# zhengchen1999/DOVE

Measured on AMD Instinct MI355X. Metric: SR frames/s (33x720x1280 4x one-step, whole job), higher is better.
Workload: dtype bf16; 1 GPU; synthetic 33x720x1280 HR clip (LR 180x320, 4x), one-step t=399, CogVideoX1.5-5B VAE + 42-layer DiT random-init, 1 clip per GPU (BASELINE configs[1]); weight_sums=True, vae_streams=2, variant=headline (bf16)

## Files before the change

### dove_amd/csrc/graph.hip

```cpp
#include <dlfcn.h>
#include <math.h>
#include <stdio.h>
#include <stdlib.h>
#include <string.h>

#include <algorithm>
#include <map>
#include <string>
#include <unordered_map>
#include <vector>

#include "common.h"
#include "../../include/dove_hip.h"
#include "ctx_access.h"

namespace {

#define CHK(expr)            \
  do {                       \
    const int rc__ = (expr); \
    if (rc__ != 0) return rc__; \
  } while (0)
#define HIPCHK(expr)                                                              \
  do {                                                                            \
// ... 689 lines not shown
      if (k) ++active;
    }
    return active;
  }
  int r = 0;
  for (int i = 0; i < nb; ++i) {
    const int s = fb[i].first, e = fb[i].second, n = e - s;
    const int spare = (world - r) - (nb - i);
    int head; bool can;
    if (enc) { head = (n % 2) + 4 * ((n - n % 2) / 8); can = n - (n % 2) >= 8 && (n - n % 2) % 8 == 0; }
    else { head = n - 1; can = n >= 2; }
    if (spare >= 1 && can) {
      const bool odd = n % 2 == 1;
      (*out)[r].push_back({s, s + head, odd ? 1 : 2, r + 1, true});
      (*out)[r + 1].push_back({s + head, e, 2, r, false});
      r += 2;
    } else {
      (*out)[r].push_back({s, e, 0, -1, false});
      r += 1;
    }
  }
  return r;
}
int piece_out_frames(const dove_ctx* c, bool enc, int t, int role) {
  if (role == 0) return enc ? enc_batch_frames(c, t) : dec_batch_frames(c, t);
  for (int i = 0; i < n_temporal_stages(c); ++i) {
    if (enc) t = t > 1 ? (t % 2 ? 1 + (t - 1) / 2 : t / 2) : 1;
    else t = role == 1 ? 2 * t - 1 : 2 * t;
  }
  return t;
}
struct RankPlan { std::vector<Piece> mine; std::vector<int> out_first; int active = 1; int total_out = 0; std::vector<int> rank_first, rank_count; };
void rank_plan(const dove_ctx* c, bool enc, int n, RankPlan* rp) {
  std::vector<std::pair<int, int>> fb;
  frame_batches(n, enc ? c->cfg.vae_enc_batch : c->cfg.vae_dec_batch, &fb);
  std::vector<std::vector<Piece>> plan;
  rp->active = plan_pieces(fb, c->nranks, enc, &plan);
  rp->rank_first.assign(c->nranks, 0); rp->rank_count.assign(c->nranks, 0);
  int f = 0;
  for (int r = 0; r < c->nranks; ++r) {
    rp->rank_first[r] = f;
    for (auto& pc : plan[r]) {
      const int k = piece_out_frames(c, enc, pc.e - pc.s, pc.role);
      if (r == c->rank) { rp->mine.push_back(pc); rp->out_first.push_back(f); }
      rp->rank_count[r] += k;
      f += k;
    }
  }
  rp->total_out = f;
}
void set_piece(dove_ctx* c, const Piece* pc) {
  c->piece_role = pc ? pc->role : 0; c->piece_partner = pc ? pc->partner : -1; c->piece_lower = pc ? pc->lower : false;
}
int norm_silu(dove_ctx* c, const Tensor& x, float* fused_stats, const std::string& name, const Tensor* zq, Tensor* out, void* stream) {
  const float eps = c->cfg.vae_norm_eps;
  float* stats = fused_stats;
  const int nb = c->nb, Ti = x.T / nb;
  if (c->piece_partner >= 0) {
    hipStream_t s = (hipStream_t)stream;
    double* sums = (double*)fused_stats;
    if (!sums) {
      sums = (double*)c->arena.alloc(64 * sizeof(double));
      DOVE_CHECK_ARG(sums, "workspace exhausted (GroupNorm sums)");
      CHK(dove_groupnorm_sums_bf16(x.p, x.elems() / x.C, (long long)x.H * x.W, x.C, gn_scratch(c), c->gn_ws_rows, sums, stream));
    }
    double* msg = (double*)c->arena.alloc(3 * 72 * sizeof(double));
    DOVE_CHECK_ARG(msg, "workspace exhausted (GroupNorm pair message)");
    double *mine = msg, *theirs = msg + 72, *tot = msg + 144;
    hipLaunchKernelGGL(gn_msg_kernel, dim3(1), dim3(128), 0, s, sums, (double)(x.elems() / 32), mine);
    CHK(pair_exchange(c, c->piece_partner, c->piece_lower, mine, theirs, 65 * sizeof(double), stream));
    hipLaunchKernelGGL(gn_add_kernel, dim3(1), dim3(128), 0, s, c->piece_lower ? mine : theirs, c->piece_lower ? theirs : mine, tot);
    c->arena.release(sums);
    stats = (float*)c->arena.alloc(64 * 4);
    CHK(dove_groupnorm_finalize_sums(tot, 0.0, eps, stats, stream));
    c->arena.release(msg);
  } else if (!stats) {
    stats = (float*)c->arena.alloc((size_t)nb * 64 * 4);
    CHK(dove_groupnorm_stats_nb_bf16(x.p, nb, x.elems() / x.C / nb, (long long)x.H * x.W, x.C, eps, gn_scratch(c), c->gn_ws_rows, stats, stream));
  }
  const auto& gb = c->aff.at(name);
  CHK(alloc_t(c, x.T, x.H, x.W, x.C, out));
  if (!zq) {
    CHK(dove_groupnorm_apply_nb_bf16(x.p, out->p, nb, Ti, x.H, x.W, x.C, stats, gb.first, gb.second, 1, nullptr, 0, 0, 0, 0, nullptr, stream));
  } else {
    Tensor yb;
    CHK(conv(c, *zq, c->pc.at(name + ".yb"), ConvOpt(), &yb, stream));
    const int ratio = x.H / zq->H;
    int sshift = 0;
    while ((1 << sshift) < ratio) ++sshift;
    std::vector<int> tmap;
    spatial_norm_tmap(Ti, zq->T / nb, &tmap);
    CHK(dove_groupnorm_apply_nb_bf16(x.p, out->p, nb, Ti, x.H, x.W, x.C, stats, gb.first, gb.second, 1, yb.p, zq->T / nb, yb.H, yb.W, sshift,
                                     tmap.data(), stream));
    free_t(c, yb);
  }
  c->arena.release(stats);
  return 0;
}
int resnet(dove_ctx* c, Tensor* x, float** xstats, const std::string& name, const Tensor* zq, void* stream, int tdup = 0) {
  const float eps = c->cfg.vae_norm_eps;
  Tensor h1, h, h2, y;
  CHK(norm_silu(c, *x, *xstats, name + ".norm1", zq, &h1, stream));
  float* hs = nullptr;
  ConvOpt o1; o1.gn_eps = eps; o1.gn_stats = &hs; o1.tdup = tdup;
  CHK(cconv(c, h1, true, name + ".conv1", o1, &h, stream));
  CHK(norm_silu(c, h, hs, name + ".norm2", zq, &h2, stream));
  free_t(c, h);
  Tensor sc = *x;
  bool own_sc = false;
  auto it = c->pc.find(name + ".conv_shortcut");
  if (it != c->pc.end()) { CHK(conv(c, *x, it->second, ConvOpt(), &sc, stream)); own_sc = true; }
  float* ys = nullptr;
  ConvOpt o2; o2.resid = sc.p; o2.ldr = sc.C; o2.gn_eps = eps; o2.gn_stats = &ys;
  CHK(cconv(c, h2, true, name + ".conv2", o2, &y, stream));
  if (own_sc) free_t(c, sc);
  free_t(c, *x);
  *x = y; *xstats = ys;
  return 0;
}
void clear_caches(dove_ctx* c);
struct StageGuard {
  dove_ctx* c;
  explicit StageGuard(dove_ctx* ctx) : c(ctx) {
    if (c && c->depth++ == 0) {
      clear_caches(c); c->arena.reset(); c->halo_recv = c->halo_send = false; c->nb = 1; set_piece(c, nullptr);
      c->ev_next = 0; c->halo_posted.clear(); c->halo_record.clear(); c->halo_sent = false;
      c->vae_multi = false;
    }
  }
  ~StageGuard() { if (c) --c->depth; }
};

int encoder(dove_ctx* c, const Tensor& x, Tensor* out, void* stream) {
  const auto& cf = c->cfg;
  Tensor h; float* hs = nullptr;
  Tensor xin = x;
  CHK(cconv(c, xin, false, c->pc.count("encoder.conv_in.taps") ? "encoder.conv_in.taps" : "encoder.conv_in", ConvOpt(), &h, stream));
  char nm[128];
  const int n_tdown = n_temporal_stages(c);
  for (int i = 0; i < cf.vae_num_blocks; ++i) {
    for (int j = 0; j < cf.vae_layers_per_block; ++j) { snprintf(nm, sizeof nm, "encoder.down_blocks.%d.resnets.%d", i, j); CHK(resnet(c, &h, &hs, nm, nullptr, stream)); }
    if (i < cf.vae_num_blocks - 1) {
      snprintf(nm, sizeof nm, "encoder.down_blocks.%d.downsamplers.0", i);
      if (hs) { c->arena.release(hs); hs = nullptr; }
      Tensor p = h;
      const int Ti = h.T / c->nb;
      if (i < n_tdown && Ti > 1) {
        const int To = Ti % 2 ? 1 + (Ti - 1) / 2 : Ti / 2;
        CHK(alloc_t(c, c->nb * To, h.H, h.W, h.C, &p));
        CHK(dove_avgpool_time_nb_bf16(h.p, c->nb, Ti, (long long)h.H * h.W * h.C, p.p, stream));
        free_t(c, h);
      }
      ConvOpt od; od.stride = 2; od.pad_h = 0; od.pad_w = 0; od.nb = c->nb;
      Tensor d;
      CHK(conv(c, p, c->pc.at(nm), od, &d, stream));
      free_t(c, p);
      h = d;
    }
  }
  for (int j = 0; j < 2; ++j) { snprintf(nm, sizeof nm, "encoder.mid_block.resnets.%d", j); CHK(resnet(c, &h, &hs, nm, nullptr, stream)); }
  Tensor n;
  CHK(norm_silu(c, h, hs, "encoder.norm_out", nullptr, &n, stream));
  free_t(c, h);
  CHK(cconv(c, n, true, "encoder.conv_out", ConvOpt(), out, stream));
  return 0;
}
int decoder(dove_ctx* c, const Tensor& z, Tensor* out, void* stream) {
  const auto& cf = c->cfg;
  Tensor h; float* hs = nullptr;
// ... 1065 lines not shown
```

### dove_amd/lib.py

```python
from __future__ import annotations

import ctypes as C
import os

import torch

_HERE = os.path.dirname(os.path.abspath(__file__))
LIB_PATH = os.path.join(_HERE, "libdove_hip.so")
_lib = None

F32, BF16, U8 = 0, 1, 2
METRIC_PSNR, METRIC_SSIM, METRIC_RGB_TO_Y = 1, 2, 4
COLORFIX_WAVELET, COLORFIX_ADAIN, COLORFIX_CLAMP = 1, 2, 1
YUV_444, YUV_422, YUV_420, YUV_MONO = 0, 1, 2, 3
YUV_SITING_LEFT, YUV_SITING_CENTRE = 0, 1
VIDEO_RGB_U8, VIDEO_YUV = 0, 1
RESIZE_BILINEAR, RESIZE_BICUBIC, RESIZE_AREA = 0, 1, 2
ACT_NONE, ACT_RELU, ACT_SIGMOID, ACT_TANH = 0, 1, 2, 3


class ConvDesc(C.Structure):
    _fields_ = [
        ("struct_size", C.c_uint), ("reserved", C.c_uint),
        ("x", C.c_void_p), ("cache", C.c_void_p), ("w", C.c_void_p), ("bias", C.c_void_p),
# ... 65 lines not shown
                ("x", C.c_void_p), ("w", C.c_void_p), ("bias", C.c_void_p), ("scale", C.c_void_p), ("shift", C.c_void_p), ("out", C.c_void_p),
                ("n", C.c_int), ("h", C.c_int), ("w_in", C.c_int), ("cin", C.c_int), ("cout", C.c_int), ("kh", C.c_int), ("kw", C.c_int),
                ("stride", C.c_int), ("act", C.c_int), ("out_mul", C.c_float), ("ldx", C.c_longlong), ("ldo", C.c_longlong)]

    def __init__(self, *a, **k):
        super().__init__(*a, **k)
        self.struct_size = C.sizeof(Conv2dF32Args)


class ConvnetConvF32Args(C.Structure):
    _fields_ = [("struct_size", C.c_uint), ("reserved", C.c_uint),
                ("x", C.c_void_p), ("w", C.c_void_p), ("bias", C.c_void_p), ("out", C.c_void_p),
                ("n", C.c_int), ("h", C.c_int), ("w_in", C.c_int), ("cin", C.c_int), ("cout", C.c_int), ("kh", C.c_int), ("kw", C.c_int),
                ("stride", C.c_int), ("pad_h", C.c_int), ("pad_w", C.c_int), ("relu", C.c_int), ("reserved2", C.c_int),
                ("ldx", C.c_longlong), ("ldo", C.c_longlong)]

    def __init__(self, *a, **k):
        super().__init__(*a, **k)
        self.struct_size = C.sizeof(ConvnetConvF32Args)


class ResnetConvF32Args(C.Structure):
    _fields_ = [("struct_size", C.c_uint), ("reserved", C.c_uint),
                ("x", C.c_void_p), ("w", C.c_void_p), ("bias", C.c_void_p), ("residual", C.c_void_p), ("out", C.c_void_p),
                ("n", C.c_int), ("h", C.c_int), ("w_in", C.c_int), ("cin", C.c_int), ("cout", C.c_int), ("k", C.c_int),
                ("stride", C.c_int), ("pool", C.c_int), ("relu", C.c_int), ("reserved2", C.c_int),
                ("ldx", C.c_longlong), ("ldr", C.c_longlong), ("ldo", C.c_longlong)]

    def __init__(self, *a, **k):
        super().__init__(*a, **k)
        self.struct_size = C.sizeof(ResnetConvF32Args)


class PreNoise(C.Structure):
    _fields_ = [("eps", C.c_void_p), ("eps_dtype", C.c_int), ("sqrt_alpha", C.c_float), ("sqrt_one_minus_alpha", C.c_float)]


OPT_VAE_TILING, OPT_VAE_SAMPLE_HEIGHT, OPT_VAE_SAMPLE_WIDTH, OPT_DIT_LINEAR_MXFP8, OPT_DIT_ATTN_MXFP8, OPT_WEIGHT_SUMS, OPT_VAE_STREAMS = 1, 2, 3, 4, 5, 6, 7
STAT_HALO_PREPOSTED, STAT_HALO_BLOCKING, STAT_HALO_SENT, STAT_HALO_COMMUNICATORS = 100, 101, 102, 103


_VP, _I, _LL, _F = C.c_void_p, C.c_int, C.c_longlong, C.c_float
_ULL, _PI, _PLL = C.c_ulonglong, C.POINTER(C.c_int), C.POINTER(C.c_longlong)
XFER_FN = C.CFUNCTYPE(C.c_int, C.c_void_p, C.c_int, C.c_void_p, C.c_size_t, C.c_void_p)
GROUP_FN = C.CFUNCTYPE(C.c_int, C.c_void_p, C.c_void_p)

SIGNATURES = {
    "dove_conv_igemm_bf16": [C.POINTER(ConvDesc), _VP],
    "dove_groupnorm_stats_bf16": [_VP, _LL, _LL, _I, _F, _VP, _I, _VP, _VP],
    "dove_groupnorm_finalize_partials": [_VP, _LL, C.c_double, _F, _VP, _VP, _VP],
    "dove_groupnorm_stats_nb_bf16": [_VP, _I, _LL, _LL, _I, _F, _VP, _I, _VP, _VP],
    "dove_groupnorm_finalize_partials_nb": [_VP, _LL, _I, C.c_double, _F, _VP, C.c_size_t, _VP, _VP],
    "dove_groupnorm_apply_nb_bf16": [_VP, _VP, _I, _I, _I, _I, _I, _VP, _VP, _VP, _I, _VP, _I, _I, _I, _I, C.POINTER(C.c_int), _VP],
    "dove_avgpool_time_nb_bf16": [_VP, _I, _I, _LL, _VP, _VP],
    "dove_groupnorm_sums_bf16": [_VP, _LL, _LL, _I, _VP, _I, _VP, _VP],
    "dove_groupnorm_finalize_sums": [_VP, C.c_double, _F, _VP, _VP],
    "dove_groupnorm_sums_from_partials": [_VP, _LL, _VP, _VP, _VP],
    "dove_groupnorm_apply_bf16": [_VP, _VP, _I, _I, _I, _I, _VP, _VP, _VP, _I, _VP, _I, _I, _I, C.POINTER(C.c_int), _VP],
    "dove_layernorm_modulate_bf16": [_VP, _VP, _LL, _I, _F, _VP, _VP, _VP, _LL, _VP],
    "dove_qkv_post_bf16": [_VP, _LL, _LL, _I, _I, _I, _VP, _VP, _VP, _VP, _VP, _VP, _F, _F, _VP, _VP, _VP, _I, _VP, _VP],
    "dove_vt_quad_swap_bf16": [_VP, _LL, _LL, _VP],
    "dove_ulysses_place_bf16": [_VP, _VP, _VP, C.POINTER(C.c_longlong), _I, _I, _LL, _LL, _VP, _VP, _VP, _VP, _VP],
    "dove_cl_im2col3x3_from_ncthw": [_VP, _I, _I, _I, _I, _I, _I, _F, _F, _VP, _VP],
    "dove_conv_out_gather": [_VP, _LL, _I, _I, _I, _I, _VP, _F, _F, _F, _F, _VP, _I, _VP],
    "dove_attention_fwd_bf16": [_VP, _VP, _VP, _VP, _LL, _LL, _I, _I, _LL, _VP, _VP],
    "dove_qkv_post_mxfp8": [_VP, _LL, _LL, _I, _I, _I, _VP, _VP, _VP, _VP, _VP, _VP, _F, _F, _VP, _VP, _VP, _VP, _VP],
    "dove_attention_fwd_mxfp8": [_VP, _VP, _VP, _VP, _VP, _LL, _LL, _I, _I, _LL, _VP],
    "dove_cl_from_ncthw": [_VP, _I, _I, _LL, _I, _F, _F, _VP, _VP],
    "dove_ncthw_from_cl": [_VP, _LL, _I, _LL, _F, _F, _F, _F, _VP, _I, _VP],
    "dove_avgpool_time_bf16": [_VP, _I, _LL, _VP, _VP],
    "dove_posterior_sample": [_VP, _LL, _I, _LL, _VP, _I, _VP, _I, _VP],
    "dove_axpby": [_VP, _VP, _VP, _I, _LL, _F, _F, _VP],
    "dove_patchify": [_VP, _I, _I, _I, _I, _I, _I, _I, _VP, _LL, _VP],
    "dove_unpatchify": [_VP, _LL, _I, _I, _I, _I, _I, _I, _VP, _I, _VP],
    "dove_gemv_bf16": [_VP, _VP, _VP, _I, _I, _I, _VP, _VP],
    "dove_blend_edge_bf16": [_VP, _VP, _I, _I, _I, _I, _I, _I, _I, _I, _VP],
    "dove_preprocess_u8": [_VP, _I, _I, _I, _I, _I, _I, _I, _VP, _I, _VP],
    "dove_postprocess_u8": [_VP, _I, _I, _I, _I, _I, _I, _I, _VP, _VP],
    "dove_rmsnorm_bf16": [_VP, _VP, _LL, _I, _F, _VP, _VP],
    "dove_gated_gelu_bf16": [_VP, _VP, _LL, _I, _VP],
    "dove_attention_bias_bf16": [_VP, _VP, _VP, _LL, _VP, _VP, _LL, _I, _I, _I, _VP],
    "dove_mx_quant_bf16": [_VP, _LL, _I, _VP, _VP, _VP],
    "dove_create": [_I, C.POINTER(ModelConfig), C.POINTER(_VP)],
    "dove_set_weight": [_VP, C.c_char_p, _VP, C.POINTER(C.c_longlong), _I, _I],
    "dove_finalize_weights": [_VP],
    "dove_set_workspace": [_VP, _VP, C.c_size_t],
    "dove_vae_encode": [_VP, _VP, _I, _I, _I, _I, _VP, _I, _VP],
    "dove_dit_forward": [_VP, _VP, _I, _I, _I, _I, _VP, _I, _I, C.POINTER(DitAux), _VP, _I, _VP],
    "dove_vae_decode": [_VP, _VP, _I, _I, _I, _I, _F, _I, _VP, _I, _VP],
    "dove_sr_clip": [_VP, _VP, _I, _I, _I, _I, _VP, _I, _VP, _I, _I, _F, _F, C.POINTER(DitAux), C.POINTER(PreNoise), _VP, _I, _VP],
    "dove_set_option": [_VP, _I, _LL],
    "dove_comm_unique_id": [_VP],
    "dove_comm_init": [_VP, _VP, _I, _I],
    "dove_comm_init_custom": [_VP, _I, _I, XFER_FN, XFER_FN, _VP],
    "dove_comm_set_group": [_VP, GROUP_FN, GROUP_FN],
    "dove_shard_frames": [_VP, _I, _I, C.POINTER(C.c_int), C.POINTER(C.c_int)],
    "dove_conv_out_gather_cl": [_VP, _LL, _I, _I, _I, _I, _VP, _VP, _I, _VP],
    "dove_tile_gather_bf16": [_VP, _I, _I, _I, _I, _I, _I, _I, _I, C.POINTER(C.c_int), C.POINTER(C.c_int), _I, _VP, _VP],
    "dove_linear_mxfp8": [_VP, _VP, _VP, _VP, _VP, _VP, _VP, _VP, _LL, _I, _I, _LL, _LL, _LL, _I, _VP],
    "dove_fr_metrics": [C.POINTER(ImageView), C.POINTER(ImageView), _I, _I, _I, _I, _I, _VP, C.c_size_t, _VP, _VP],
    "dove_color_fix": [C.POINTER(ImageView), _F, _F, C.POINTER(ImageView), _F, _F, _I, _I, _I, _I, _I, C.POINTER(ImageView), _VP,
                       C.c_size_t, _VP],
    "dove_rgb_to_yuv_u8": [C.POINTER(ImageView), _I, _I, _I, C.POINTER(YuvFormat), _VP, _VP],
    "dove_yuv_to_rgb_u8": [_VP, _I, _I, _I, C.POINTER(YuvFormat), _VP, _VP],
    "dove_plan_padding": [_I, _I, _I, _PI, _PI, _PI],
    "dove_plan_output_size": [_I, _I, _I, _PI, _PI],
# ... 188 lines not shown
```

### dove_amd/ops.py

```python
from __future__ import annotations

import ctypes as C
import math
from dataclasses import dataclass

import numpy as np
import torch

from . import lib as L


def _ru(x: int, m: int) -> int:
    return (x + m - 1) // m * m


@dataclass
class PackedConv:
    w: torch.Tensor
    bias: torch.Tensor | None
    kt: int
    kh: int
    kw: int
    cin: int
    cin_pad: int
    cout: int
    cout_pad: int
    w_first: torch.Tensor | None = None
    w_sub: torch.Tensor | None = None
    w_pair: torch.Tensor | None = None

    @property
    def cout_store(self) -> int:
        return _ru(self.cout, 4)


def pack_conv(weight: torch.Tensor, bias: torch.Tensor | None, device, *, sub: bool = True, pair: bool = False) -> PackedConv:
    w = weight.detach()
    if w.dim() == 2:
        w = w[:, :, None, None, None]
    elif w.dim() == 4:
        w = w[:, :, None]
    cout, cin, kt, kh, kw = w.shape
    cin_pad = _ru(cin, 32) if cin <= 32 or cin % 64 else cin
    cout_pad = _ru(cout, 32)
    wp = torch.zeros(kt * kh * kw, cout_pad, cin_pad, dtype=torch.bfloat16, device=device)
    wp[:, :cout, :cin] = w.to(device=device, dtype=torch.float32).permute(2, 3, 4, 0, 1).reshape(kt * kh * kw, cout, cin).to(torch.bfloat16)
    bp = None
    if bias is not None:
        bp = torch.zeros(cout_pad, dtype=torch.float32, device=device)
        bp[:cout] = bias.detach().to(device=device, dtype=torch.float32)
    wp = wp.contiguous()
    w_first = None
    if kt == 3:
        t = wp.float().view(3, kh * kw, cout_pad, cin_pad)
        s01 = t[0] + t[1]
        w_first = torch.stack([s01, s01 + t[2]]).to(torch.bfloat16).contiguous()
# ... 225 lines not shown
                                               L.stream_ptr()), "dove_groupnorm_stats_bf16")
    return stats


def groupnorm_sums(x: torch.Tensor) -> torch.Tensor:
    L.require_cuda(x)
    assert x.dtype == torch.bfloat16
    Cc = x.shape[-1]
    sums = torch.empty(32, 2, dtype=torch.float64, device=x.device)
    ws = _ws(x.device, _gn_rows_needed(x, x.shape[0] if x.dim() == 4 else 1))
    L.check(L.load().dove_groupnorm_sums_bf16(L.ptr(x), x.numel() // Cc, _frame_pix(x), Cc, L.ptr(ws), ws.numel() // 64, L.ptr(sums),
                                              L.stream_ptr()), "dove_groupnorm_sums_bf16")
    return sums


def groupnorm_sums_of(x: torch.Tensor) -> torch.Tensor:
    rows = getattr(x, "gn_rows", None)
    if rows is None:
        return groupnorm_sums(x)
    sums = torch.empty(32, 2, dtype=torch.float64, device=x.device)
    L.check(L.load().dove_groupnorm_sums_from_partials(L.ptr(rows), rows.shape[0], L.ptr(_ws(x.device)), L.ptr(sums), L.stream_ptr()),
            "dove_groupnorm_sums_from_partials")
    return sums


def groupnorm_from_sums(sums: torch.Tensor, count: float, eps: float) -> torch.Tensor:
    L.require_cuda(sums)
    assert sums.dtype == torch.float64 and (sums.shape == (32, 2) if count is not None else sums.numel() == 65)
    stats = torch.empty(32, 2, dtype=torch.float32, device=sums.device)
    L.check(L.load().dove_groupnorm_finalize_sums(L.ptr(sums.contiguous()), 0.0 if count is None else float(count), eps, L.ptr(stats), L.stream_ptr()),
            "dove_groupnorm_finalize_sums")
    return stats


def groupnorm_apply(x, stats, gamma, beta, *, silu=True, yb=None, sshift=0, tmap=None, out=None, nb=1):
    L.require_cuda(x, stats, gamma, beta, yb, out)
    T, H, W, Cc = x.shape
    assert T % nb == 0 and stats.numel() == nb * 64
    T //= nb
    if out is None:
        out = torch.empty_like(x)
    Tz = hz = wz = 0
    tm = None
    if yb is not None:
        assert yb.dtype == torch.bfloat16 and yb.shape[-1] == 2 * Cc and tmap is not None and len(tmap) == T and yb.shape[0] % nb == 0
        Tz, hz, wz = yb.shape[0] // nb, yb.shape[1], yb.shape[2]
        tm = (C.c_int * T)(*tmap)
    L.check(L.load().dove_groupnorm_apply_nb_bf16(L.ptr(x), L.ptr(out), nb, T, H, W, Cc, L.ptr(stats), L.ptr(gamma), L.ptr(beta),
                                                  int(silu), L.ptr(yb), Tz, hz, wz, sshift, tm, L.stream_ptr()),
            "dove_groupnorm_apply_nb_bf16")
    return out


def layernorm_modulate(x, gamma, beta, eps, mod=None, split=0, out=None):
    L.require_cuda(x, gamma, beta, mod, out)
    assert x.dtype == torch.bfloat16 and x.dim() == 2
    if out is None:
        out = torch.empty_like(x)
    if mod is not None:
        assert mod.dtype == torch.float32 and mod.shape == (2, 2, x.shape[1])
    L.check(L.load().dove_layernorm_modulate_bf16(L.ptr(x), L.ptr(out), x.shape[0], x.shape[1], eps, L.ptr(gamma),
                                                  L.ptr(beta), L.ptr(mod), split, L.stream_ptr()),
            "dove_layernorm_modulate_bf16")
    return out


def qkv_post(qkv, N, Npad, heads, text_len, gq, bq, gk, bk, cos, sin, qscale, eps, Qh, Kh, Vt, v_order=1, norm2=None):
    L.require_cuda(qkv, gq, bq, gk, bk, cos, sin, Qh, Kh, Vt, norm2)
    if norm2 is not None:
        assert norm2.dtype == torch.float32 and norm2.shape == (heads, 2) and norm2.is_contiguous()
    L.check(L.load().dove_qkv_post_bf16(L.ptr(qkv), N, Npad, heads, 64, text_len, L.ptr(gq), L.ptr(bq), L.ptr(gk), L.ptr(bk),
                                        L.ptr(cos), L.ptr(sin), qscale, eps, L.ptr(Qh), L.ptr(Kh), L.ptr(Vt), v_order, L.ptr(norm2),
                                        L.stream_ptr()), "dove_qkv_post_bf16")


def vt_quad_swap(Vt):
    L.require_cuda(Vt)
    assert Vt.is_contiguous()
    L.check(L.load().dove_vt_quad_swap_bf16(L.ptr(Vt), Vt.numel() // Vt.shape[-1], Vt.shape[-1], L.stream_ptr()), "dove_vt_quad_swap_bf16")
    return Vt


def ulysses_place(rq, rk, rv, counts, hloc, N, Npad, Qh, Kh, Vt, norm2_out=None):
    L.require_cuda(rq, rk, rv, Qh, Kh, Vt, norm2_out)
    if norm2_out is not None:
        assert norm2_out.dtype == torch.float32 and norm2_out.shape == (hloc, 2)
    cnt = (C.c_longlong * len(counts))(*[int(c) for c in counts])
    L.check(L.load().dove_ulysses_place_bf16(L.ptr(rq), L.ptr(rk), L.ptr(rv), cnt, len(counts), hloc, N, Npad, L.ptr(Qh), L.ptr(Kh), L.ptr(Vt),
                                             L.ptr(norm2_out), L.stream_ptr()), "dove_ulysses_place_bf16")


def attention(Qh, Kh, Vt, N, Npad, heads, out, norm2=None):
    L.require_cuda(Qh, Kh, Vt, out, norm2)
    if norm2 is not None:
        assert norm2.dtype == torch.float32 and norm2.shape == (heads, 2) and norm2.is_contiguous()
    L.check(L.load().dove_attention_fwd_bf16(L.ptr(Qh), L.ptr(Kh), L.ptr(Vt), L.ptr(out), N, Npad, heads, 64, out.shape[1], L.ptr(norm2),
                                             L.stream_ptr()), "dove_attention_fwd_bf16")
    return out


def attention_head_paths(norm2, heads=None):
    lib = L.load()
    if norm2 is None:
        host, n = None, int(heads)
    else:
        host = norm2.detach().float().cpu().contiguous()
# ... 1436 lines not shown
```

### dove_amd/vae.py

```python
from __future__ import annotations

import math
import re

import torch

from . import ops
from .config import AttrDict


def frame_batches(num_frames: int, batch: int):
    n = max(num_frames // batch, 1)
    rem = num_frames % batch
    return [(batch * i + (0 if i == 0 else rem), min(batch * (i + 1) + rem, num_frames)) for i in range(n)]


def spatial_norm_tmap(t_f: int, t_z: int):
    if t_f > 1 and t_f % 2 == 1:
        if t_z == 1:
            return [0] * t_f
        return [0] + [1 + ((t - 1) * (t_z - 1)) // (t_f - 1) for t in range(1, t_f)]
    return [(t * t_z) // t_f for t in range(t_f)]


# ... 107 lines not shown
        self.use_slicing = False

    def enable_tiling(self, *a, **k):
        self.use_tiling = True

    def disable_tiling(self):
        self.use_tiling = False

    def to(self, *a, **k):
        return self

    def _cconv(self, x, name, cache, **kw):
        pc = self.pc[name]
        kw["weight_sums"] = self.weight_sums
        nb = self._nb
        if pc.kt == 1:
            return ops.conv(x, pc, nb=nb, **kw)
        k = pc.kt - 1
        x5 = x.view(nb, x.shape[0] // nb, *x.shape[1:])
        fetch = getattr(cache, "fetch", None)
        if fetch:
            assert nb == 1, "tiles are not batched under the halo exchange"
            prev = fetch(name, (k,) + tuple(x.shape[1:]), x.device)
            prev, pair = (None if prev is None else prev[None]), True
        else:
            prev, pair = cache.get(name, (None, False))
        events = getattr(cache, "events", None)
        if events is not None and name in events:
            cache.stream.wait_event(events[name])
            prev.record_stream(cache.stream)
        tdup = kw.get("tdup", 0)
        if tdup == 1 and prev is not None and not pair:
            kw["tdup"] = 0
        if x5.shape[1] >= k:
            new = x5[:, -k:]
        else:
            pad = prev if prev is not None else x5[:, :1].expand(-1, k, -1, -1, -1)
            new = torch.cat([pad, x5], dim=1)[:, -k:].contiguous()
        if events is not None:
            events[name] = torch.cuda.Event()
            events[name].record(cache.stream)
        if fetch:
            cache.publish(name, new[0])
        else:
            cache[name] = (new, bool(tdup) and x5.shape[1] >= k)
        if prev is not None and nb == 1:
            prev = prev[0]
        return ops.conv(x, pc, cache=prev, nb=nb, **kw)

    _gn_hook = None
    _piece_role = None
    _nb = 1

    def _norm_silu(self, x, name, zq=None):
        nb = self._nb
        if self._gn_hook is not None:
            stats = self._gn_hook(x)
        else:
            stats = ops.groupnorm_stats_of(x, self.eps, nb)
        g, b = self.aff[name]
        if zq is None:
            return ops.groupnorm_apply(x, stats, g, b, silu=True, nb=nb)
        yb = ops.conv(zq, self.pc[name + ".yb"])
        ratio = x.shape[1] // zq.shape[1]
        assert x.shape[1] == zq.shape[1] * ratio and x.shape[2] == zq.shape[2] * ratio and ratio & (ratio - 1) == 0
        return ops.groupnorm_apply(x, stats, g, b, silu=True, yb=yb, sshift=ratio.bit_length() - 1,
                                   tmap=spatial_norm_tmap(x.shape[0] // nb, zq.shape[0] // nb), nb=nb)

    def _resnet(self, x, name, cache, zq=None, tdup=0):
        h = self._norm_silu(x, name + ".norm1", zq)
        h = self._cconv(h, name + ".conv1", cache, gn_eps=self.eps, tdup=tdup)
        h = self._norm_silu(h, name + ".norm2", zq)
        if name + ".conv_shortcut" in self.pc:
            x = ops.conv(x, self.pc[name + ".conv_shortcut"])
        return self._cconv(h, name + ".conv2", cache, resid=x, gn_eps=self.eps)

    def _downsample(self, x, name, compress_time):
        if compress_time:
            x = ops.avgpool_time(x, self._nb)
        return ops.conv(x, self.pc[name], stride=2, pad=(0, 0), nb=self._nb)

    def _upsample(self, x, name, compress_time):
        T = x.shape[0] // self._nb
        if compress_time and self._piece_role is not None:
            tmode, t_out = (2, 2 * T - 1) if self._piece_role == "head" else (1, 2 * T)
        elif compress_time and T > 1:
            tmode, t_out = (2, 2 * T - 1) if T % 2 == 1 else (1, 2 * T)
        else:
            tmode, t_out = 0, T
        return ops.conv(x, self.pc[name], up=1, tmode=tmode, t_out=t_out, pad=(1, 1), gn_eps=self.eps, nb=self._nb,
                        weight_sums=self.weight_sums), tmode

    def _encoder(self, x, cache, split_in=False):
        h = self._cconv(x, "encoder.conv_in.taps" if split_in and self._conv_in_split else "encoder.conv_in", cache)
        nb = len(self.boc)
        for i in range(nb):
            for j in range(self.layers):
                h = self._resnet(h, f"encoder.down_blocks.{i}.resnets.{j}", cache)
            if i < nb - 1:
                h = self._downsample(h, f"encoder.down_blocks.{i}.downsamplers.0", i < self.n_tdown)
        for j in range(2):
            h = self._resnet(h, f"encoder.mid_block.resnets.{j}", cache)
        h = self._norm_silu(h, "encoder.norm_out")
        return self._cconv(h, "encoder.conv_out", cache)

    def _decoder(self, z, cache, split_out=False):
        h = self._cconv(z, "decoder.conv_in", cache)
        for j in range(2):
            h = self._resnet(h, f"decoder.mid_block.resnets.{j}", cache, zq=z)
        nb = len(self.boc)
        tdup = 0
        for i in range(nb):
            for j in range(self.layers + 1):
                h = self._resnet(h, f"decoder.up_blocks.{i}.resnets.{j}", cache, zq=z, tdup=tdup if j == 0 else 0)
            if i < nb - 1:
                h, tdup = self._upsample(h, f"decoder.up_blocks.{i}.upsamplers.0", i < self.n_tdown)
        h = self._norm_silu(h, "decoder.norm_out", zq=z)
        if split_out and self._conv_out_split:
            return self._cconv(h, "decoder.conv_out.taps", cache, out_f32=True)
        return self._cconv(h, "decoder.conv_out", cache)

    def _tiling_params(self):
        c = self.config
        down = 2 ** (len(self.boc) - 1)
        smin_h, smin_w = c.get("sample_height", 480) // 2, c.get("sample_width", 720) // 2
        return dict(smin_h=smin_h, smin_w=smin_w, lmin_h=int(smin_h / down), lmin_w=int(smin_w / down), of_h=1 / 6, of_w=1 / 5)

# ... 183 lines not shown
```

### include/dove_hip.h

```cpp
#ifndef DOVE_HIP_H
#define DOVE_HIP_H

#include <stddef.h>

#ifdef __cplusplus
extern "C" {
#endif

#define DOVE_ABI_VERSION 15

#define DOVE_F32 0
#define DOVE_BF16 1

const char* dove_last_error(void);
int dove_abi_version(void);
int dove_device_info(int dev, char* name, int name_len, int* cu_count, long long* total_mem);

typedef struct dove_conv_desc {
  unsigned int struct_size;
  unsigned int reserved;
  const void* x;
  const void* cache;
  const void* w;
  const float* bias;
  const void* resid;
  const float* gate;
  void* out;
  int t_in, h_in, w_in, cin;
  int t_out, h_out, w_out, cout_pad, cout_store;
  int kt, kh, kw, stride, pad_h, pad_w, up, tmode, act;
  long long ldo, ldr, gate_split;
  float* gn_partial;
  int out_f32;
  int nb;
  long long cache_stride;
  const void* w_first;
  const void* w_sub;
  const void* w_pair;
  int tdup;
  int reserved2;
} dove_conv_desc;
int dove_conv_igemm_bf16(const dove_conv_desc* d, void* stream);
const char* dove_conv_kernel_name(const dove_conv_desc* d);
int dove_conv_partial_launches(const dove_conv_desc* d);
long long dove_conv_gn_partial_rows(const dove_conv_desc* d);
int dove_groupnorm_finalize_partials(const float* partial, long long rows, double count, float eps, void* ws, float* stats,
                                     void* stream);

int dove_groupnorm_stats_bf16(const void* x, long long npix, long long frame_pix, int C, float eps, void* partial_ws, int ws_blocks,
                              float* stats, void* stream);
int dove_groupnorm_sums_bf16(const void* x, long long npix, long long frame_pix, int C, void* partial_ws, int ws_blocks, double* sums,
                             void* stream);
int dove_groupnorm_finalize_sums(const double* sums, double count, float eps, float* stats, void* stream);
int dove_groupnorm_sums_from_partials(const float* partial, long long rows, void* ws, double* sums, void* stream);
int dove_groupnorm_apply_bf16(const void* x, void* y, int T, int H, int W, int C, const float* stats,
                              const float* gamma, const float* beta, int silu, const void* yb, int hz, int wz,
                              int sshift, const int* tmap, void* stream);

int dove_groupnorm_stats_nb_bf16(const void* x, int nb, long long npix, long long frame_pix, int C, float eps, void* partial_ws,
                                 int ws_blocks, float* stats, void* stream);
int dove_groupnorm_finalize_partials_nb(const float* partial, long long rows, int nb, double count, float eps, void* ws, size_t ws_bytes,
                                        float* stats, void* stream);
int dove_groupnorm_apply_nb_bf16(const void* x, void* y, int nb, int T, int H, int W, int C, const float* stats, const float* gamma,
                                 const float* beta, int silu, const void* yb, int Tz, int hz, int wz, int sshift, const int* tmap,
                                 void* stream);
int dove_avgpool_time_nb_bf16(const void* x, int nb, int T, long long frame_elems, void* y, void* stream);

int dove_layernorm_modulate_bf16(const void* x, void* y, long long rows, int D, float eps, const float* gamma,
                                 const float* beta, const float* mod, long long split, void* stream);

int dove_qkv_post_bf16(const void* qkv, long long N, long long Npad, int heads, int head_dim, int text_len,
                       const float* gq, const float* bq, const float* gk, const float* bk, const float* cosT,
                       const float* sinT, float qscale, float eps, void* Qh, void* Kh, void* Vt, int v_order, float* norm2, void* stream);
int dove_vt_quad_swap_bf16(void* Vt, long long rows, long long Npad, void* stream);
int dove_ulysses_place_bf16(const void* rq, const void* rk, const void* rv, const long long* counts, int world, int hloc, long long N,
                            long long Npad, void* Qh, void* Kh, void* Vt, float* norm2_out, void* stream);

int dove_attention_fwd_bf16(const void* Qh, const void* Kh, const void* Vt, void* O, long long N, long long Npad,
                            int heads, int head_dim, long long ldo, float* norm2, void* stream);
int dove_attention_head_paths(const float* norm2_host, int heads, int* path);
const char* dove_attention_path_name(int path);

int dove_cl_from_ncthw(const void* x, int dtype, int C, long long npix, int Cp, float scale, float shift, void* y,
                       void* stream);
int dove_ncthw_from_cl(const void* x, long long ld, int C, long long npix, float scale, float shift, float lo,
                       float hi, void* y, int dtype, void* stream);
int dove_cl_im2col3x3_from_ncthw(const void* x, int dtype, int C, int T, int H, int W, int Cp, float scale, float shift, void* y,
                                 void* stream);
int dove_conv_out_gather(const float* p, long long ldp, int T, int H, int W, int C, const float* bias, float scale, float shift, float lo,
                         float hi, void* y, int dtype, void* stream);
int dove_avgpool_time_bf16(const void* x, int T, long long frame_elems, void* y, void* stream);
int dove_posterior_sample(const void* moments, long long ld, int latent_channels, long long npix, const void* noise,
                          int noise_dtype, void* out, int out_dtype, void* stream);
int dove_axpby(const void* x, const void* y, void* out, int dtype, long long n, float a, float b, void* stream);
int dove_patchify(const void* x, int dtype, int T, int C, int H, int W, int pt, int p, void* tokens, long long ld,
                  void* stream);
int dove_unpatchify(const void* tokens, long long ld, int T, int C, int H, int W, int pt, int p, void* y, int dtype,
                    void* stream);
int dove_conv_out_gather_cl(const float* p, long long ldp, int T, int H, int W, int C, const float* bias, void* y, int ldy, void* stream);
int dove_tile_gather_bf16(const void* x, int H, int W, int C, int t0, int nt, int th, int tw, int nb, const int* oy, const int* ox,
                          int im2col_cin, void* out, void* stream);
int dove_blend_edge_bf16(const void* a, void* b, int T, int Ha, int Wa, int Hb, int Wb, int ld, int extent, int axis,
                         void* stream);
int dove_preprocess_u8(const void* frames, int F0, int H0, int W0, int pad_f, int pad_h, int pad_w, int upscale, void* out,
                       int out_dtype, void* stream);
int dove_postprocess_u8(const void* video, int dtype, int F, int H, int W, int Fo, int Ho, int Wo, void* out, void* stream);

#define DOVE_U8 2
#define DOVE_METRIC_PSNR 1
#define DOVE_METRIC_SSIM 2
#define DOVE_METRIC_RGB_TO_Y 4
typedef struct dove_image_view {
  const void* data;
  int dtype;
  int reserved;
  long long sn, sc, sh, sw;
} dove_image_view;
size_t dove_fr_metrics_workspace_bytes(int n, int h, int w);
int dove_fr_metrics(const dove_image_view* pred, const dove_image_view* ref, int n, int channels, int h, int w, int flags, void* ws,
// ... 338 lines not shown
```

Baseline: 34.71 frames/s.

## Fuse GroupNorm-apply with 1x1 conv shortcut in VAE resnet blocks

Adds a kernel that applies GroupNorm (with optional spatial-norm modulation) and SiLU to the input while also computing the 1x1 conv_shortcut from the same input tile with MFMA, keeping the shortcut weights in LDS. The input is then read once instead of twice, and the separate shortcut conv launch goes away. The resnet block now frees the original input early. Only the channel pairs (256,128) and (128,256) with nb==1 are covered. The kernel is double-buffered and persistent, with one workgroup per CU, which may limit occupancy.

```diff
diff --git a/dove_amd/csrc/gn_shortcut.hip b/dove_amd/csrc/gn_shortcut.hip
--- /dev/null
+++ b/dove_amd/csrc/gn_shortcut.hip
@@ -0,0 +1,248 @@
+#include <type_traits>
+
+#include "common.h"
+#include "../../include/dove_hip.h"
+
+struct GnShortcutArgs {
+  const bf16_t* x; bf16_t* y; const float* stats; const float* gamma; const float* beta; const bf16_t* yb;
+  const bf16_t* w; const float* bias; bf16_t* s;
+  long long ldy, lds;
+  unsigned npix;
+  int ntiles;
+  int T, H, W, hz, wz, sshift, act;
+  int tmap[32];
+};
+
+namespace gnsc {
+constexpr int NT = 512;
+constexpr int TILE = 64;
+__device__ __forceinline__ int swz(int c, int row) { return (c & ~15) | ((c ^ row) & 15); }
+}
+
+template <int CIN, int COUT, bool YB>
+__global__ __launch_bounds__(gnsc::NT) void gn_shortcut_kernel(const GnShortcutArgs a) {
+  using namespace gnsc;
+  constexpr int CPR = CIN / 8;
+  constexpr int CPR_LOG = CIN == 256 ? 5 : 4;
+  constexpr int NSUB = NT / CPR;
+  constexpr int NP = TILE / NSUB;
+  constexpr int CB = COUT / 128;
+  constexpr int KS = CIN / 16;
+  constexpr int ROWB = CIN * 2;
+  constexpr int XT = TILE * ROWB;
+  constexpr int WB = COUT * ROWB;
+  static_assert(NP >= 1 && CB >= 1 && WB == 65536, "gn_shortcut: unsupported shape");
+  extern __shared__ __attribute__((aligned(16))) char smem[];
+  int* tmap_s = (int*)(smem + WB + 2 * XT);
+
+  const int tid = threadIdx.x, lane = tid & 63;
+  const int wave = __builtin_amdgcn_readfirstlane(tid >> 6);
+  const int q = tid & (CPR - 1), sub = tid >> CPR_LOG;
+
+  for (int i = tid; i < COUT * CPR; i += NT) {
+    const int row = i >> CPR_LOG, c = i & (CPR - 1);
+    *(uint4*)(smem + row * ROWB + swz(c, row) * 16) = *(const uint4*)(a.w + (long long)row * CIN + c * 8);
+  }
+  if (tid < 32) tmap_s[tid] = a.tmap[tid];
+  __syncthreads();
+
+  constexpr int cpg = CIN / 32;
+  float sc[8], sh[8];
+#pragma unroll
+  for (int e = 0; e < 8; ++e) {
+    const int ch = q * 8 + e, g = ch / cpg;
+    const float mean = a.stats[g * 2], rstd = a.stats[g * 2 + 1];
+    sc[e] = rstd * a.gamma[ch];
+    sh[e] = a.beta[ch] - mean * sc[e];
+  }
+
+  const int hi = lane >> 5, l31 = lane & 31;
+  const int pb = wave >> 2, cb0 = (wave & 3) * CB;
+  const int xrow = pb * 32 + l31;
+  f32x4 bias[CB][4];
+#pragma unroll
+  for (int i = 0; i < CB; ++i)
+#pragma unroll
+    for (int g = 0; g < 4; ++g) {
+      bias[i][g] = f32x4{0.f, 0.f, 0.f, 0.f};
+      if (a.bias) bias[i][g] = *(const f32x4*)(a.bias + (cb0 + i) * 32 + 8 * g + 4 * hi);
+    }
+
+  const unsigned HW = (unsigned)a.H * (unsigned)a.W;
+  const int nfull = (int)(a.npix / TILE);
+
+  auto load_tile = [&](int tile, uint4* xr, uint4* yr, uint4* br) {
+    const unsigned p0 = (unsigned)tile * TILE;
+    int t = 0, h = 0, w = 0;
+    if (YB) {
+      t = (int)(p0 / HW);
+      const unsigned r = p0 - (unsigned)t * HW;
+      h = (int)(r / (unsigned)a.W);
+      w = (int)(r - (unsigned)h * (unsigned)a.W) + sub;
+    }
+#pragma unroll
+    for (int u = 0; u < NP; ++u) {
+      const unsigned p = min(p0 + sub + u * NSUB, a.npix - 1);
+      xr[u] = *(const uint4*)(a.x + (long long)p * CIN + q * 8);
+      if (YB) {
+        while (w >= a.W) { w -= a.W; if (++h == a.H) { h = 0; ++t; } }
+        const long long zrow = ((long long)tmap_s[min(t, a.T - 1)] * a.hz + (h >> a.sshift)) * a.wz;
+        const bf16_t* yb = a.yb + (zrow + (w >> a.sshift)) * (2 * CIN) + q * 8;
+        yr[u] = *(const uint4*)yb;
+        br[u] = *(const uint4*)(yb + CIN);
+        w += NSUB;
+      }
+    }
+  };
+
+  auto step = [&](auto fullc, int tile, int buf, const uint4* xc, const uint4* yc, const uint4* bc, uint4* xn, uint4* yn, uint4* bn) {
+    constexpr bool FULL = decltype(fullc)::value;
+    char* xt = smem + WB + buf * XT;
+    const unsigned p0 = (unsigned)tile * TILE;
+#pragma unroll
+    for (int u = 0; u < NP; ++u) {
+      const int row = sub + u * NSUB;
+      *(uint4*)(xt + row * ROWB + swz(q, row) * 16) = xc[u];
+    }
+    __syncthreads();
+    const int nxt = tile + (int)gridDim.x;
+    if (FULL && nxt < nfull) load_tile(nxt, xn, yn, bn);
+
+#pragma unroll
+    for (int u = 0; u < NP; ++u) {
+      const unsigned p = p0 + sub + u * NSUB;
+      if (FULL || p < a.npix) {
+        float f[8];
+        unpack8(xc[u], f);
+#pragma unroll
+        for (int e = 0; e < 8; ++e) f[e] = f[e] * sc[e] + sh[e];
+        if (YB) {
+          float fy[8], fb[8];
+          unpack8(yc[u], fy);
+          unpack8(bc[u], fb);
+#pragma unroll
+          for (int e = 0; e < 8; ++e) f[e] = f[e] * fy[e] + fb[e];
+        }
+        if (a.act) {
+#pragma unroll
+          for (int e = 0; e < 8; ++e) f[e] = silu_f(f[e]);
+        }
+        *(uint4*)(a.y + (long long)p * a.ldy + q * 8) = pack8(f);
+      }
+    }
+
+    f32x16 acc[CB];
+#pragma unroll
+    for (int i = 0; i < CB; ++i)
+#pragma unroll
+      for (int r = 0; r < 16; ++r) acc[i][r] = 0.f;
+#pragma unroll
+    for (int ks = 0; ks < KS; ++ks) {
+      const int chunk = ks * 2 + hi;
+      const bf16x8 xf = *(const bf16x8*)(xt + xrow * ROWB + swz(chunk, xrow) * 16);
+      bf16x8 wf[CB];
+#pragma unroll
+      for (int i = 0; i < CB; ++i) {
+        const int wrow = (cb0 + i) * 32 + l31;
+        wf[i] = *(const bf16x8*)(smem + wrow * ROWB + swz(chunk, wrow) * 16);
+      }
+#pragma unroll
+      for (int i = 0; i < CB; ++i) acc[i] = __builtin_amdgcn_mfma_f32_32x32x16_bf16(wf[i], xf, acc[i], 0, 0, 0);
+    }
+    const unsigned p = p0 + xrow;
+    if (FULL || p < a.npix) {
+      bf16_t* srow = a.s + (long long)p * a.lds;
+#pragma unroll
+      for (int i = 0; i < CB; ++i)
+#pragma unroll
+        for (int g = 0; g < 4; ++g) {
+          const int cb = (cb0 + i) * 32 + 8 * g + 4 * hi;
+          float v[4];
+#pragma unroll
+          for (int e = 0; e < 4; ++e) v[e] = acc[i][g * 4 + e];
+          if (a.bias) {
+#pragma unroll
+            for (int e = 0; e < 4; ++e) v[e] += bias[i][g][e];
+          }
+          uint2 o;
+          o.x = pack_bf2(v[0], v[1]);
+          o.y = pack_bf2(v[2], v[3]);
+          *(uint2*)(srow + cb) = o;
+        }
+    }
+  };
+
+  uint4 x0[NP], y0[NP], b0[NP], x1[NP], y1[NP], b1[NP];
+  int tile = blockIdx.x;
+  if (tile < nfull) load_tile(tile, x0, y0, b0);
+  asm volatile("s_waitcnt vmcnt(0)" ::: "memory");
+  while (tile < nfull) {
+    step(std::true_type{}, tile, 0, x0, y0, b0, x1, y1, b1);
+    tile += gridDim.x;
+    if (tile >= nfull) break;
+    step(std::true_type{}, tile, 1, x1, y1, b1, x0, y0, b0);
+    tile += gridDim.x;
+  }
+  if (tile < a.ntiles) {
+    __syncthreads();
+    load_tile(tile, x0, y0, b0);
+    step(std::false_type{}, tile, 0, x0, y0, b0, x1, y1, b1);
+  }
+}
+
+static int gnsc_cu_count() {
+  static std::atomic<int> cus[DOVE_MAX_DEVICES] = {};
+  int dev = 0;
+  (void)hipGetDevice(&dev);
+  int n = (dev >= 0 && dev < DOVE_MAX_DEVICES) ? cus[dev].load(std::memory_order_relaxed) : 0;
+  if (!n) {
+    n = 256;
+    (void)hipDeviceGetAttribute(&n, hipDeviceAttributeMultiprocessorCount, dev);
+    if (dev >= 0 && dev < DOVE_MAX_DEVICES) cus[dev].store(n, std::memory_order_relaxed);
+  }
+  return n;
+}
+
+template <int CIN, int COUT, bool YB>
+static int launch_gn_shortcut(const GnShortcutArgs& a, hipStream_t s) {
+  constexpr int lds = COUT * CIN * 2 + 2 * gnsc::TILE * CIN * 2 + 32 * 4;
+  static PerDeviceOnce attr_set;
+  if (auto once_ = attr_set.guard()) (void)hipFuncSetAttribute((const void*)gn_shortcut_kernel<CIN, COUT, YB>, hipFuncAttributeMaxDynamicSharedMemorySize, lds);
+  const int cus = gnsc_cu_count();
+  const unsigned grid = a.ntiles > cus ? (unsigned)cus : (unsigned)a.ntiles;
+  hipLaunchKernelGGL((gn_shortcut_kernel<CIN, COUT, YB>), dim3(grid), dim3(gnsc::NT), lds, s, a);
+  DOVE_CHECK_LAUNCH("dove_groupnorm_apply_shortcut_bf16");
+  return DOVE_OK;
+}
+
+extern "C" int dove_groupnorm_apply_shortcut_bf16(const void* x, void* y, long long ldy, int nb, int T, int H, int W, int C, const float* stats,
+                                                  const float* gamma, const float* beta, int silu, const void* yb, int Tz, int hz, int wz,
+                                                  int sshift, const int* tmap, const void* w, const float* bias, int Cout, void* s,
+                                                  long long lds, void* stream) {
+  DOVE_CHECK_ARG(x && y && stats && gamma && beta && w && s, "groupnorm_apply_shortcut: null pointer");
+  DOVE_CHECK_ARG(nb == 1, "groupnorm_apply_shortcut: one GroupNorm scope per call (nb = %d)", nb);
+  DOVE_CHECK_ARG((C == 256 && Cout == 128) || (C == 128 && Cout == 256),
+                 "groupnorm_apply_shortcut: (Cin, Cout) = (%d, %d) is not one of (256, 128), (128, 256)", C, Cout);
+  DOVE_CHECK_ARG(T > 0 && T <= 32 && H > 0 && W > 0, "groupnorm_apply_shortcut: need 0 < T <= 32 frames per batch (got %d), H, W > 0", T);
+  DOVE_CHECK_ARG((long long)T * H * W < (1ll << 31) - 64, "groupnorm_apply_shortcut: too many pixels");
+  DOVE_CHECK_ARG(ldy >= C && ldy % 8 == 0, "groupnorm_apply_shortcut: ldy (%lld) must be a multiple of 8 and >= C", ldy);
+  DOVE_CHECK_ARG(lds >= Cout && lds % 4 == 0, "groupnorm_apply_shortcut: lds (%lld) must be a multiple of 4 and >= Cout", lds);
+  GnShortcutArgs a;
+  a.x = (const bf16_t*)x; a.y = (bf16_t*)y; a.stats = stats; a.gamma = gamma; a.beta = beta; a.yb = (const bf16_t*)yb;
+  a.w = (const bf16_t*)w; a.bias = bias; a.s = (bf16_t*)s; a.ldy = ldy; a.lds = lds;
+  a.npix = (unsigned)((long long)T * H * W);
+  a.ntiles = (int)((a.npix + gnsc::TILE - 1) / gnsc::TILE);
+  a.T = T; a.H = H; a.W = W; a.hz = hz; a.wz = wz; a.sshift = sshift; a.act = silu;
+  for (int i = 0; i < 32; ++i) a.tmap[i] = 0;
+  if (yb) {
+    DOVE_CHECK_ARG(tmap, "groupnorm_apply_shortcut: spatial norm needs a frame map");
+    DOVE_CHECK_ARG(sshift >= 0 && sshift <= 8 && (hz << sshift) >= H && (wz << sshift) >= W, "groupnorm_apply_shortcut: latent grid too small");
+    for (int i = 0; i < T; ++i) {
+      DOVE_CHECK_ARG(tmap[i] >= 0 && tmap[i] < Tz, "groupnorm_apply_shortcut: frame map entry %d (%d) outside the %d latent frames", i, tmap[i], Tz);
+      a.tmap[i] = tmap[i];
+    }
+  }
+  hipStream_t st = (hipStream_t)stream;
+  if (C == 256) return yb ? launch_gn_shortcut<256, 128, true>(a, st) : launch_gn_shortcut<256, 128, false>(a, st);
+  return yb ? launch_gn_shortcut<128, 256, true>(a, st) : launch_gn_shortcut<128, 256, false>(a, st);
+}
diff --git a/dove_amd/csrc/graph.hip b/dove_amd/csrc/graph.hip
--- a/dove_amd/csrc/graph.hip
+++ b/dove_amd/csrc/graph.hip
@@ -765,7 +765,17 @@
 void set_piece(dove_ctx* c, const Piece* pc) {
   c->piece_role = pc ? pc->role : 0; c->piece_partner = pc ? pc->partner : -1; c->piece_lower = pc ? pc->lower : false;
 }
-int norm_silu(dove_ctx* c, const Tensor& x, float* fused_stats, const std::string& name, const Tensor* zq, Tensor* out, void* stream) {
+bool gn_shortcut_enabled() {
+  const char* e = getenv("DOVE_OPT_GN_SHORTCUT");
+  return !(e && e[0] == '0' && e[1] == 0);
+}
+bool gn_shortcut_fuses(const dove_ctx* c, const Tensor& x, const Packed& pc) {
+  const bool shape = (x.C == 256 && pc.cout_pad == 128) || (x.C == 128 && pc.cout_pad == 256);
+  return c->nb == 1 && gn_shortcut_enabled() && shape && pc.kt * pc.kh * pc.kw == 1 && pc.cin_pad == x.C && pc.cout_store() == pc.cout_pad &&
+         x.T <= 32 && (long long)x.T * x.H * x.W < (1ll << 31) - 64;
+}
+int norm_silu(dove_ctx* c, const Tensor& x, float* fused_stats, const std::string& name, const Tensor* zq, Tensor* out, void* stream,
+              const Packed* shortcut = nullptr, Tensor* sc = nullptr) {
   const float eps = c->cfg.vae_norm_eps;
   float* stats = fused_stats;
   const int nb = c->nb, Ti = x.T / nb;
@@ -793,8 +803,15 @@
   }
   const auto& gb = c->aff.at(name);
   CHK(alloc_t(c, x.T, x.H, x.W, x.C, out));
+  const bool fuse = shortcut && sc && gn_shortcut_fuses(c, x, *shortcut);
+  if (fuse) CHK(alloc_t(c, x.T, x.H, x.W, shortcut->cout_store(), sc));
   if (!zq) {
-    CHK(dove_groupnorm_apply_nb_bf16(x.p, out->p, nb, Ti, x.H, x.W, x.C, stats, gb.first, gb.second, 1, nullptr, 0, 0, 0, 0, nullptr, stream));
+    if (fuse) {
+      CHK(dove_groupnorm_apply_shortcut_bf16(x.p, out->p, x.C, 1, Ti, x.H, x.W, x.C, stats, gb.first, gb.second, 1, nullptr, 0, 0, 0, 0, nullptr,
+                                             shortcut->w, shortcut->bias, shortcut->cout_pad, sc->p, sc->C, stream));
+    } else {
+      CHK(dove_groupnorm_apply_nb_bf16(x.p, out->p, nb, Ti, x.H, x.W, x.C, stats, gb.first, gb.second, 1, nullptr, 0, 0, 0, 0, nullptr, stream));
+    }
   } else {
     Tensor yb;
     CHK(conv(c, *zq, c->pc.at(name + ".yb"), ConvOpt(), &yb, stream));
@@ -803,8 +820,13 @@
     while ((1 << sshift) < ratio) ++sshift;
     std::vector<int> tmap;
     spatial_norm_tmap(Ti, zq->T / nb, &tmap);
-    CHK(dove_groupnorm_apply_nb_bf16(x.p, out->p, nb, Ti, x.H, x.W, x.C, stats, gb.first, gb.second, 1, yb.p, zq->T / nb, yb.H, yb.W, sshift,
-                                     tmap.data(), stream));
+    if (fuse) {
+      CHK(dove_groupnorm_apply_shortcut_bf16(x.p, out->p, x.C, 1, Ti, x.H, x.W, x.C, stats, gb.first, gb.second, 1, yb.p, zq->T, yb.H, yb.W, sshift,
+                                             tmap.data(), shortcut->w, shortcut->bias, shortcut->cout_pad, sc->p, sc->C, stream));
+    } else {
+      CHK(dove_groupnorm_apply_nb_bf16(x.p, out->p, nb, Ti, x.H, x.W, x.C, stats, gb.first, gb.second, 1, yb.p, zq->T / nb, yb.H, yb.W, sshift,
+                                       tmap.data(), stream));
+    }
     free_t(c, yb);
   }
   c->arena.release(stats);
@@ -813,21 +835,27 @@
 int resnet(dove_ctx* c, Tensor* x, float** xstats, const std::string& name, const Tensor* zq, void* stream, int tdup = 0) {
   const float eps = c->cfg.vae_norm_eps;
   Tensor h1, h, h2, y;
-  CHK(norm_silu(c, *x, *xstats, name + ".norm1", zq, &h1, stream));
+  Tensor sc = *x;
+  bool own_sc = false;
+  auto it = c->pc.find(name + ".conv_shortcut");
+  if (it != c->pc.end()) {
+    Tensor fsc;
+    CHK(norm_silu(c, *x, *xstats, name + ".norm1", zq, &h1, stream, &it->second, &fsc));
+    if (fsc.p) { free_t(c, *x); sc = fsc; own_sc = true; }
+  } else {
+    CHK(norm_silu(c, *x, *xstats, name + ".norm1", zq, &h1, stream));
+  }
   float* hs = nullptr;
   ConvOpt o1; o1.gn_eps = eps; o1.gn_stats = &hs; o1.tdup = tdup;
   CHK(cconv(c, h1, true, name + ".conv1", o1, &h, stream));
   CHK(norm_silu(c, h, hs, name + ".norm2", zq, &h2, stream));
   free_t(c, h);
-  Tensor sc = *x;
-  bool own_sc = false;
-  auto it = c->pc.find(name + ".conv_shortcut");
-  if (it != c->pc.end()) { CHK(conv(c, *x, it->second, ConvOpt(), &sc, stream)); own_sc = true; }
+  if (it != c->pc.end() && !own_sc) { CHK(conv(c, *x, it->second, ConvOpt(), &sc, stream)); own_sc = true; }
   float* ys = nullptr;
   ConvOpt o2; o2.resid = sc.p; o2.ldr = sc.C; o2.gn_eps = eps; o2.gn_stats = &ys;
   CHK(cconv(c, h2, true, name + ".conv2", o2, &y, stream));
   if (own_sc) free_t(c, sc);
-  free_t(c, *x);
+  if (x->p) free_t(c, *x);
   *x = y; *xstats = ys;
   return 0;
 }
diff --git a/dove_amd/lib.py b/dove_amd/lib.py
--- a/dove_amd/lib.py
+++ b/dove_amd/lib.py
@@ -141,6 +141,8 @@
     "dove_groupnorm_stats_nb_bf16": [_VP, _I, _LL, _LL, _I, _F, _VP, _I, _VP, _VP],
     "dove_groupnorm_finalize_partials_nb": [_VP, _LL, _I, C.c_double, _F, _VP, C.c_size_t, _VP, _VP],
     "dove_groupnorm_apply_nb_bf16": [_VP, _VP, _I, _I, _I, _I, _I, _VP, _VP, _VP, _I, _VP, _I, _I, _I, _I, C.POINTER(C.c_int), _VP],
+    "dove_groupnorm_apply_shortcut_bf16": [_VP, _VP, _LL, _I, _I, _I, _I, _I, _VP, _VP, _VP, _I, _VP, _I, _I, _I, _I, C.POINTER(C.c_int),
+                                           _VP, _VP, _I, _VP, _LL, _VP],
     "dove_avgpool_time_nb_bf16": [_VP, _I, _I, _LL, _VP, _VP],
     "dove_groupnorm_sums_bf16": [_VP, _LL, _LL, _I, _VP, _I, _VP, _VP],
     "dove_groupnorm_finalize_sums": [_VP, C.c_double, _F, _VP, _VP],
diff --git a/dove_amd/ops.py b/dove_amd/ops.py
--- a/dove_amd/ops.py
+++ b/dove_amd/ops.py
@@ -2,6 +2,7 @@
 
 import ctypes as C
 import math
+import os
 from dataclasses import dataclass
 
 import numpy as np
@@ -333,6 +334,55 @@
     return out
 
 
+GN_SHORTCUT_SHAPES = ((256, 128), (128, 256))
+
+
+def gn_shortcut_enabled() -> bool:
+    return os.environ.get("DOVE_OPT_GN_SHORTCUT", "1") != "0"
+
+
+def groupnorm_apply_shortcut(x, stats, gamma, beta, pc: PackedConv, *, silu=True, yb=None, sshift=0, tmap=None, out=None, s_out=None, nb=1):
+    T, H, W, Cc = x.shape
+    fused = (x.is_cuda and nb == 1 and gn_shortcut_enabled() and (Cc, pc.cout_pad) in GN_SHORTCUT_SHAPES and pc.kt * pc.kh * pc.kw == 1
+             and pc.cin_pad == Cc and pc.cout_store == pc.cout_pad and T <= 32 and T * H * W < (1 << 31) - 64)
+    if not fused:
+        if out is not None and out.shape[-1] != Cc:
+            out[..., :Cc] = groupnorm_apply(x, stats, gamma, beta, silu=silu, yb=yb, sshift=sshift, tmap=tmap, nb=nb)
+            y = out
+        else:
+            y = groupnorm_apply(x, stats, gamma, beta, silu=silu, yb=yb, sshift=sshift, tmap=tmap, out=out, nb=nb)
+        kw = {} if s_out is None else dict(out=s_out, ldo=s_out.shape[-1])
+        return y, conv(x, pc, **kw)
+    L.require_cuda(x, stats, gamma, beta, yb, out, s_out)
+    assert x.dtype == torch.bfloat16 and stats.numel() == 64
+    if out is None:
+        out = torch.empty_like(x)
+    if s_out is None:
+        s_out = torch.empty(T, H, W, pc.cout_store, dtype=torch.bfloat16, device=x.device)
+    assert out.shape[:3] == x.shape[:3] and out.dtype == torch.bfloat16 and s_out.shape[:3] == x.shape[:3] and s_out.dtype == torch.bfloat16
+    Tz = hz = wz = 0
+    tm = None
+    if yb is not None:
+        assert yb.dtype == torch.bfloat16 and yb.shape[-1] == 2 * Cc and tmap is not None and len(tmap) == T
+        Tz, hz, wz = yb.shape[0], yb.shape[1], yb.shape[2]
+        tm = (C.c_int * T)(*tmap)
+    if _profiler is not None:
+        e0, e1 = torch.cuda.Event(enable_timing=True), torch.cuda.Event(enable_timing=True)
+        e0.record()
+    L.check(L.load().dove_groupnorm_apply_shortcut_bf16(L.ptr(x), L.ptr(out), out.shape[-1], 1, T, H, W, Cc, L.ptr(stats), L.ptr(gamma),
+                                                        L.ptr(beta), int(silu), L.ptr(yb), Tz, hz, wz, sshift, tm, L.ptr(pc.w), L.ptr(pc.bias),
+                                                        pc.cout_pad, L.ptr(s_out), s_out.shape[-1], L.stream_ptr()),
+            "dove_groupnorm_apply_shortcut_bf16")
+    if _profiler is not None:
+        e1.record()
+        flops = 2.0 * T * H * W * pc.cout * pc.cin
+        _profiler.append(((pc.cin, pc.cout, 1), flops, e0, e1, "gn_shortcut_kernel", flops))
+    if getattr(s_out, "gn_stats", None) is not None:
+        s_out.gn_stats = None
+        s_out.gn_rows = None
+    return out, s_out
+
+
 def layernorm_modulate(x, gamma, beta, eps, mod=None, split=0, out=None):
     L.require_cuda(x, gamma, beta, mod, out)
     assert x.dtype == torch.bfloat16 and x.dim() == 2
diff --git a/dove_amd/vae.py b/dove_amd/vae.py
--- a/dove_amd/vae.py
+++ b/dove_amd/vae.py
@@ -183,27 +183,30 @@
     _piece_role = None
     _nb = 1
 
-    def _norm_silu(self, x, name, zq=None):
+    def _norm_silu(self, x, name, zq=None, shortcut=None):
         nb = self._nb
         if self._gn_hook is not None:
             stats = self._gn_hook(x)
         else:
             stats = ops.groupnorm_stats_of(x, self.eps, nb)
         g, b = self.aff[name]
-        if zq is None:
-            return ops.groupnorm_apply(x, stats, g, b, silu=True, nb=nb)
-        yb = ops.conv(zq, self.pc[name + ".yb"])
-        ratio = x.shape[1] // zq.shape[1]
-        assert x.shape[1] == zq.shape[1] * ratio and x.shape[2] == zq.shape[2] * ratio and ratio & (ratio - 1) == 0
-        return ops.groupnorm_apply(x, stats, g, b, silu=True, yb=yb, sshift=ratio.bit_length() - 1,
-                                   tmap=spatial_norm_tmap(x.shape[0] // nb, zq.shape[0] // nb), nb=nb)
+        kw = {}
+        if zq is not None:
+            ratio = x.shape[1] // zq.shape[1]
+            assert x.shape[1] == zq.shape[1] * ratio and x.shape[2] == zq.shape[2] * ratio and ratio & (ratio - 1) == 0
+            kw = dict(yb=ops.conv(zq, self.pc[name + ".yb"]),
+                      sshift=ratio.bit_length() - 1, tmap=spatial_norm_tmap(x.shape[0] // nb, zq.shape[0] // nb))
+        if shortcut is not None:
+            return ops.groupnorm_apply_shortcut(x, stats, g, b, self.pc[shortcut], silu=True, nb=nb, **kw)
+        return ops.groupnorm_apply(x, stats, g, b, silu=True, nb=nb, **kw)
 
     def _resnet(self, x, name, cache, zq=None, tdup=0):
-        h = self._norm_silu(x, name + ".norm1", zq)
+        if name + ".conv_shortcut" in self.pc:
+            h, x = self._norm_silu(x, name + ".norm1", zq, shortcut=name + ".conv_shortcut")
+        else:
+            h = self._norm_silu(x, name + ".norm1", zq)
         h = self._cconv(h, name + ".conv1", cache, gn_eps=self.eps, tdup=tdup)
         h = self._norm_silu(h, name + ".norm2", zq)
-        if name + ".conv_shortcut" in self.pc:
-            x = ops.conv(x, self.pc[name + ".conv_shortcut"])
         return self._cconv(h, name + ".conv2", cache, resid=x, gn_eps=self.eps)
 
     def _downsample(self, x, name, compress_time):
diff --git a/include/dove_hip.h b/include/dove_hip.h
--- a/include/dove_hip.h
+++ b/include/dove_hip.h
@@ -65,6 +65,10 @@
                                  const float* beta, int silu, const void* yb, int Tz, int hz, int wz, int sshift, const int* tmap,
                                  void* stream);
 int dove_avgpool_time_nb_bf16(const void* x, int nb, int T, long long frame_elems, void* y, void* stream);
+
+int dove_groupnorm_apply_shortcut_bf16(const void* x, void* y, long long ldy, int nb, int T, int H, int W, int C, const float* stats,
+                                       const float* gamma, const float* beta, int silu, const void* yb, int Tz, int hz, int wz, int sshift,
+                                       const int* tmap, const void* w, const float* bias, int Cout, void* s, long long lds, void* stream);
 
 int dove_layernorm_modulate_bf16(const void* x, void* y, long long rows, int D, float eps, const float* gamma,
                                  const float* beta, const float* mod, long long split, void* stream);
```

Result: no change. 34.87 frames/s, median of 2 (+0.5%).
